# zixunh/vipe

Hardware: AMD Instinct MI355X
Metric: dense-BA+flow update iters/s, 512x384 48-KF graph (higher is better)
Workload: dtype f16 (correlation, GRU; fp32 accumulate) + f32 geometry/BA (fp64 reduced system)

## Files before the change

### include/vipe_amd.h

```cpp
#ifndef VIPE_AMD_H
#define VIPE_AMD_H

#include <stdint.h>

#ifdef __cplusplus
extern "C" {
#endif

#define VIPE_F16 0
#define VIPE_F32 1
#define VIPE_F64 2
#define VIPE_U8 3

#define VIPE_OK 0
#define VIPE_EINVAL (-1)
#define VIPE_ENOSPACE (-2)
#define VIPE_EUNSUPPORTED (-3)

#define VIPE_PYRAMID_REFERENCE 0
#define VIPE_PYRAMID_BLOCKED 1

#define VIPE_CAM_PINHOLE 0
#define VIPE_CAM_MEI 1

// ... 174 lines not shown
int vipe_scatter_mean_rows_f16(const void* d_src, const int64_t* d_ix, void* d_out, int E, int n_out, int64_t inner,
                               void* stream);

int vipe_segment_mean_nhwc_f16(const void* d_src, int src_ctot, int src_coff, const int* d_order, const int* d_rowptr,
                               void* d_out, int n_out, int64_t rows_per_item, int C, void* stream);

int vipe_corr_sampler_forward(const void* d_in1, const void* d_in2, void* d_out, int B, int C, int H, int W, int kH,
                              int kW, int patchH, int patchW, int padH, int padW, int dilH, int dilW,
                              int dil_patchH, int dil_patchW, int dH, int dW, int dtype, void* stream);
int vipe_corr_sampler_backward(const void* d_in1, const void* d_in2, const void* d_grad_out, void* d_grad1,
                               void* d_grad2, int B, int C, int H, int W, int kH, int kW, int patchH, int patchW,
                               int padH, int padW, int dilH, int dilW, int dil_patchH, int dil_patchW, int dH,
                               int dW, int dtype, void* stream);

int vipe_corr_sampler_forward_host(const float* h_in1, const float* h_in2, float* h_out, int B, int C, int H, int W, int kH,
                                   int kW, int patchH, int patchW, int padH, int padW, int dilH, int dilW, int dil_patchH,
                                   int dil_patchW, int dH, int dW);
int vipe_corr_sampler_backward_host(const float* h_in1, const float* h_in2, const float* h_grad_out, float* h_grad1,
                                    float* h_grad2, int B, int C, int H, int W, int kH, int kW, int patchH, int patchW,
                                    int padH, int padW, int dilH, int dilW, int dil_patchH, int dil_patchW, int dH, int dW);

int vipe_nearest_neighbours(const float* d_query, int qdim, const float* d_tree, int tdim, int64_t M, int64_t N, int knn,
                            float* d_dist, int* d_idx, void* stream);

int vipe_ms_deform_attn_forward(const void* d_value, const int64_t* d_spatial_shapes, const int64_t* d_level_start_index,
                                const void* d_sampling_loc, const void* d_attn_weight, void* d_output, int64_t bs,
                                int64_t Lv, int heads, int C, int L, int64_t Lq, int P, int dtype, void* stream);
int vipe_ms_deform_attn_backward(const void* d_value, const int64_t* d_spatial_shapes, const int64_t* d_level_start_index,
                                 const void* d_sampling_loc, const void* d_attn_weight, const void* d_grad_output,
                                 void* d_grad_value, void* d_grad_sampling_loc, void* d_grad_attn_weight, int64_t bs,
                                 int64_t Lv, int heads, int C, int L, int64_t Lq, int P, int dtype, void* stream);

#define VIPE_ACT_NONE 0
#define VIPE_ACT_RELU 1
#define VIPE_ACT_SIGMOID 2
#define VIPE_ACT_TANH 3
int vipe_conv_pack_weights(const void* d_w_oihw, void* d_w_packed, int Cout, int Cin, int KH, int KW, int src_dtype,
                           void* stream);
int vipe_conv2d_nhwc_f16(const void* d_x, const void* d_w_packed, const float* d_bias, const float* d_extra,
                         void* d_y, int B, int H, int W, int Cin, int cin_total, int cin_off, int Cout,
                         int cout_total, int cout_off, int KH, int KW, int act, void* stream);

int vipe_conv_packed_dims(int Cout, int Cin, int KH, int KW, int* cout_pad, int* cin_pad, int* k_pad);

#define VIPE_CONV_PARTIAL 6
#define VIPE_CONV_ACCINIT_F32 0x100
int vipe_conv2d_fused(const void* d_x0, int x0_ctot, int x0_coff, const void* d_x1, int x1_ctot, int x1_coff,
                      int split, const void* d_w_packed, const float* d_bias, const float* d_extra, int extra_stride,
                      int extra_off, void* d_y, int y_ctot, int y_coff, void* d_y2, int y2_ctot, int y2_coff,
                      const void* d_net, int net_ctot, int net_coff, const void* d_z, float* d_fout,
                      const void* d_accinit, int ai_ctot, int ai_coff, int B, int H, int W, int Cin, int Cout, int KH,
                      int KW, int act, int mode, void* stream);

typedef struct {
  const void *corr0_w, *corr2_w, *flow0_w, *flow2_w, *gw_w, *zr_w, *q_w, *zr_s_w, *q_s_w, *heads0_w, *heads2_w, *agg2_w, *eta_w;
  const void *zr_n_w, *zr_x_w;
  const float *corr0_b, *corr2_b, *flow0_b, *flow2_b, *gw_b, *zr_b, *q_b, *heads0_b, *heads2_b, *agg2_b, *eta_b;
  const float* glo_wT;
  const float* glo_b;
} vipe_update_weights;
typedef struct {
  int E, H, W, n_src;
  const void* levels[4];
  const float* coords;
  const int* slots;
  int h2, w2, pyramid_layout;
  const void* corr;
  const void* motn;
  const void* net;
  void* net_out;
  void* xbuf;
  const void* pgate;
  void *c1, *f1, *zb, *rnet;
  void* hbuf;
  float* dw;
  float *glo, *extra;
  const int *order, *rowptr;
  void *agg, *a2;
  float* eta;
  void* side_stream;
  float* pzr;
  int gate_state;
} vipe_update_buffers;
int vipe_update_operator(const vipe_update_weights* weights, const vipe_update_buffers* buffers, void* stream);

int vipe_update_gate_state(const vipe_update_weights* weights, const vipe_update_buffers* buffers, const void* d_net,
                           int parts, void* stream);
typedef struct {
  const vipe_update_weights* weights;
  const vipe_update_buffers* buffers;
  const void* net;
  const int* bounds;
  int n_bounds;
} vipe_gate_state_job;
int vipe_update_gate_state_piece(void* user, int piece, int n_pieces, void* stream);

int vipe_glo_context(const float* d_glo_sum, const float* d_wT, const float* d_bias, float* d_extra, int E, int hw,
                     void* stream);

typedef struct {
  const void* src;
  void* dst;
  const int64_t* idx;
  int64_t src_row_pitch, dst_row_pitch;
  int64_t seg_bytes, seg_pitch;
  int n_seg;
// ... 38 lines not shown
```

### vipe_amd/csrc/conv_mfma.hip

```cpp
#include <stdlib.h>

#include <type_traits>

#include "common.cuh"

namespace {

typedef _Float16 half8 __attribute__((ext_vector_type(8)));
typedef _Float16 half4 __attribute__((ext_vector_type(4)));
typedef float float16v __attribute__((ext_vector_type(16)));
typedef float float4v __attribute__((ext_vector_type(4)));

enum Epi { EPI_PLAIN = 0, EPI_GLO = 1, EPI_ZR = 2, EPI_Q = 3, EPI_HEADS = 4, EPI_ETA = 5, EPI_PARTIAL = 6 };

struct ConvArgs {
  const half_t* x0; int x0_ctot, x0_coff;
  const half_t* x1; int x1_ctot, x1_coff;
  int split;
  const half_t* w;
  const float* bias;
  const float* extra;
  int extra_stride, extra_off;
  half_t* y; int y_ctot, y_coff;
  int B, H, W, Cin, Cin_pad, Cout, Cout_pad, KH, KW, nsteps;
// ... 686 lines not shown
        if (cout0 + tid < a.Cout) atomicAdd(a.fout + (int64_t)e * a.Cout + cout0 + tid, t);
      }
    }
  } else {
    constexpr int PITCH = BMC + 4;
    float* stage = reinterpret_cast<float*>(lds);
#pragma unroll
    for (int i = 0; i < MI; ++i)
#pragma unroll
      for (int j = 0; j < NJ; ++j)
        *reinterpret_cast<float4*>(stage + (wn * 64 + pxh + j * 16 + l16) * PITCH + i * 16 + 4 * lk) =
            make_float4(acc16[i][j][0], acc16[i][j][1], acc16[i][j][2], acc16[i][j][3]);
    __syncthreads();
    float bv[8];
#pragma unroll
    for (int q = 0; q < 8; ++q) {
      bv[q] = a.bias[co + q];
      if (a.extra && co + q < a.Cout) bv[q] += a.extra[(int64_t)e * a.extra_stride + a.extra_off + co + q];
    }
#pragma unroll
    for (int it = 0; it < NIT; ++it) {
      const int pl = pl0 + PSTEP * it;
      const int64_t m = pix_of(pl);
      if (FLAT && m < 0) continue;
      const float4 v0 = *reinterpret_cast<const float4*>(stage + pl * PITCH + ch);
      const float4 v1 = *reinterpret_cast<const float4*>(stage + pl * PITCH + ch + 4);
      const float v[8] = {v0.x + bv[0], v0.y + bv[1], v0.z + bv[2], v0.w + bv[3],
                          v1.x + bv[4], v1.y + bv[5], v1.z + bv[6], v1.w + bv[7]};
      if (a.epi == EPI_HEADS) {
        if (ch == 0)
          *reinterpret_cast<float4*>(a.fout + m * 4) =
              make_float4((float)(half_t)v[0], (float)(half_t)v[1], (float)(half_t)act_apply(v[2], VIPE_ACT_SIGMOID),
                          (float)(half_t)act_apply(v[3], VIPE_ACT_SIGMOID));
      } else if (a.epi == EPI_ETA) {
        if (ch == 0) {
          const float sp = v[0] > 20.0f ? v[0] : log1pf(__expf(v[0]));
          a.fout[m] = 0.01f * (float)(half_t)sp;
        }
      } else {
        half_t* dst = a.y + m * a.y_ctot + a.y_coff + co;
        half8 o;
#pragma unroll
        for (int q = 0; q < 8; ++q) o[q] = (half_t)act_apply(v[q], a.act);
        if (co + 8 <= a.Cout) {
          *reinterpret_cast<half8*>(dst) = o;
        } else {
          for (int q = 0; q < 8 && co + q < a.Cout; ++q) dst[q] = o[q];
        }
      }
    }
  }
}

constexpr int NRW_WBYTES = 9 * 1024;

template <bool FLAT>
__global__ __launch_bounds__(512) __attribute__((amdgpu_waves_per_eu(4, 4))) void conv_halo32_narrow_kernel(ConvArgs a) {
  extern __shared__ __align__(16) unsigned char lds[];
  const int tid = threadIdx.x, lane = tid & 63, wave = __builtin_amdgcn_readfirstlane(tid >> 6);
  const int wn = wave & 3, pxh = (wave >> 2) * 32;
  const int tile = xcd_remap(blockIdx.x, gridDim.x);
  const int xsegs = a.W / HALO_TW, tiles_per_img = FLAT ? a.f_tiles : (a.H / HALO_TH) * xsegs;
  const int e = tile / tiles_per_img, trem = tile % tiles_per_img;
  const int y0 = (trem / xsegs) * HALO_TH, x0 = (trem % xsegs) * HALO_TW;
  const int q0 = trem * (HALO_TH * HALO_TW);
  const int pitch = FLAT ? a.f_wp : HALO_PITCH, xbytes = FLAT ? a.f_xbytes : H32_XBYTES;
  const int npieces = FLAT ? a.f_pieces : H32_PIECES;
  auto pix_of = [&](int pl) -> int64_t {
    if constexpr (FLAT) return flat_pixel(q0 + pl, e, a.H, a.W, a.f_wp, a.f_hwp, a.f_magic);
    else return ((int64_t)(e * a.H + y0 + (pl >> 6))) * a.W + x0 + (pl & 63);
  };
  const int cs32 = a.Cin_pad / H32_BK, cs64 = a.Cin_pad / 64;
  const int r16 = lane >> 2, sl = lane & 3, l16 = lane & 15, lk = lane >> 4;
  const unsigned ldsW_a = lds_address(lds), ldsX_a = ldsW_a + 2 * NRW_WBYTES;
  const unsigned char* ldsW = lds;
  const unsigned char* ldsX = lds + 2 * NRW_WBYTES;
  const half_t* zp = reinterpret_cast<const half_t*>(g_zero_page);

  int xpix[H32_XP];
  const int xk = (sl ^ swzf(r16)) * 8;
#pragma unroll
  for (int i = 0; i < H32_XP; ++i) {
    const int pce = wave + 8 * i;
    const int r = pce * 16 + r16;
    if constexpr (FLAT) {
      xpix[i] = pce < npieces ? flat_pixel(q0 - pitch - 1 + r, e, a.H, a.W, a.f_wp, a.f_hwp, a.f_magic) : -1;
    } else {
      const int hy = r / HALO_PITCH, hx = r % HALO_PITCH;
      const int y = y0 + hy - 1, x = x0 + hx - 1;
      const bool ok = pce < H32_PIECES && r < HALO_ROWS && y >= 0 && y < a.H && x >= 0 && x < a.W;
      xpix[i] = ok ? (e * a.H + y) * a.W + x : -1;
    }
  }
  auto issue = [&](int c, int buf) {
    const int c0 = c * H32_BK;
    const bool s0 = c0 < a.split;
    const int ctot = s0 ? a.x0_ctot : a.x1_ctot;
    const int cb = (s0 ? a.x0_coff : a.x1_coff - a.split) + c0;
#pragma unroll
    for (int i = 0; i < H32_XP; ++i) {
      if (wave + 8 * i < npieces) {
        const bool ok = xpix[i] >= 0 && (c0 + xk < a.Cin);
        const uint64_t off = ((uint64_t)(unsigned)xpix[i] * (unsigned)ctot + (unsigned)(cb + xk)) * 2u;
        const char* src = reinterpret_cast<const char*>(s0 ? a.x0 : a.x1) + off;
        glds16(ok ? (const void*)src : (const void*)zp, ldsX_a + buf * xbytes + (wave + 8 * i) * 1024);
      }
    }
    const unsigned woff = (unsigned)(r16 * 64 + ((sl ^ swzf(r16)) << 3)) * 2u;
    const half_t* wb = a.w + ((int64_t)(wave * cs64 + (c >> 1)) * a.Cout_pad) * BK + (c & 1) * H32_BK;
    glds16_off(wb, woff, ldsW_a + buf * NRW_WBYTES + wave * 1024);
    if (wave == 0) {
      const half_t* w8 = a.w + ((int64_t)(8 * cs64 + (c >> 1)) * a.Cout_pad) * BK + (c & 1) * H32_BK;
      glds16_off(w8, woff, ldsW_a + buf * NRW_WBYTES + 8 * 1024);
    }
  };

  float4v acc[2] = {float4v{0.f, 0.f, 0.f, 0.f}, float4v{0.f, 0.f, 0.f, 0.f}};
  const int wa0 = swz32(l16, lk);
  const int Rl0 = (FLAT ? wn * HALO_TW : wn * HALO_PITCH) + pxh + l16;
  issue(0, 0);
  asm volatile("s_waitcnt vmcnt(0)" ::: "memory");
  __syncthreads();
  for (int c = 0; c < cs32; ++c) {
    if (c + 1 < cs32) issue(c + 1, (c + 1) & 1);
    const unsigned char* bw = ldsW + (c & 1) * NRW_WBYTES;
    const unsigned char* bx = ldsX + (c & 1) * xbytes;
#pragma unroll
    for (int tap = 0; tap < 9; ++tap) {
      const int rb = Rl0 + (tap / 3) * pitch + (tap % 3);
      const int xa0 = swz32(rb, lk);
      const half8 wf = *reinterpret_cast<const half8*>(bw + (wa0 + tap * 1024));
#pragma unroll
      for (int j = 0; j < 2; ++j) {
        const half8 xf = *reinterpret_cast<const half8*>(bx + (xa0 + j * 1024));
        acc[j] = __builtin_amdgcn_mfma_f32_16x16x32_f16(wf, xf, acc[j], 0, 0, 0);
      }
    }
    asm volatile("s_waitcnt vmcnt(0)" ::: "memory");
    __syncthreads();
  }
  constexpr int PITCH = 20;
  float* stage = reinterpret_cast<float*>(lds);
#pragma unroll
  for (int j = 0; j < 2; ++j)
    *reinterpret_cast<float4*>(stage + (wn * 64 + pxh + j * 16 + l16) * PITCH + 4 * lk) =
        make_float4(acc[j][0], acc[j][1], acc[j][2], acc[j][3]);
  __syncthreads();
  const int64_t m = tid < HALO_TH * HALO_TW ? pix_of(tid) : -1;
  if (tid < HALO_TH * HALO_TW && (!FLAT || m >= 0)) {
    float v[16];
#pragma unroll
    for (int q = 0; q < 4; ++q) {
      const float4 t4 = *reinterpret_cast<const float4*>(stage + tid * PITCH + 4 * q);
      v[4 * q] = t4.x; v[4 * q + 1] = t4.y; v[4 * q + 2] = t4.z; v[4 * q + 3] = t4.w;
    }
#pragma unroll
    for (int q = 0; q < 16; ++q) {
      v[q] += a.bias[q];
      if (a.extra && q < a.Cout) v[q] += a.extra[(int64_t)e * a.extra_stride + a.extra_off + q];
    }
    if (a.epi == EPI_HEADS) {
      *reinterpret_cast<float4*>(a.fout + m * 4) =
          make_float4((float)(half_t)v[0], (float)(half_t)v[1], (float)(half_t)act_apply(v[2], VIPE_ACT_SIGMOID),
                      (float)(half_t)act_apply(v[3], VIPE_ACT_SIGMOID));
    } else if (a.epi == EPI_ETA) {
      const float sp = v[0] > 20.0f ? v[0] : log1pf(__expf(v[0]));
      a.fout[m] = 0.01f * (float)(half_t)sp;
    } else {
      half_t* dst = a.y + m * a.y_ctot + a.y_coff;
      for (int q = 0; q < a.Cout; ++q) dst[q] = (half_t)act_apply(v[q], a.act);
    }
  }
}

constexpr int GLO_PITCH = 136;
constexpr size_t GLO_LDS = 256 * GLO_PITCH * 2 + 128 * 4;

__global__ __launch_bounds__(512) __attribute__((amdgpu_waves_per_eu(4, 4))) void conv1x1_glo_kernel(ConvArgs a) {
  extern __shared__ __align__(16) unsigned char lds[];
  half_t* xt = reinterpret_cast<half_t*>(lds);
  float* gacc = reinterpret_cast<float*>(lds + 256 * GLO_PITCH * 2);
  const int tid = threadIdx.x, lane = tid & 63, wave = tid >> 6;
  const int l16 = lane & 15, kg = lane >> 4;
  const int wq = wave & 3, wp = wave >> 2;
  const int HW = a.H * a.W;
  const int tpi = (HW + 255) / 256;
  const int e = blockIdx.x / tpi, p0 = (blockIdx.x % tpi) * 256;
  const int64_t pix0 = (int64_t)e * HW + p0;
  if (tid < 128) gacc[tid] = 0.0f;
#pragma unroll
  for (int it = 0; it < 8; ++it) {
    const int i = tid + 512 * it, px = i >> 4, ck = i & 15;
    half8 v = {0, 0, 0, 0, 0, 0, 0, 0};
// ... 206 lines not shown
  if (vipe_conv_packed_dims(Cout, Cin, KH, KW, &cp, &cinp, &kp) != VIPE_OK) return VIPE_EINVAL;
  VIPE_CHECK_ARG(Cin == 4 || Cin % 8 == 0);
  const int64_t total = (int64_t)kp * cp;
  pack_weights_kernel<<<(int)std::min<int64_t>((total + 255) / 256, 4096), 256, 0, as_stream(stream)>>>(
      d_w_oihw, (half_t*)d_w_packed, Cout, Cin, KH, KW, cp, cinp, kp, src_dtype == VIPE_F32, Cin == 4);
  return vipe_launch_status();
}

}

namespace {

template <typename K>
void allow_lds(K kernel, std::atomic<uint64_t>& seen, size_t bytes) {
  vipe_once_per_device(seen, [&] { (void)hipFuncSetAttribute((const void*)kernel, hipFuncAttributeMaxDynamicSharedMemorySize, (int)bytes); });
}
constexpr size_t MAX_LDS = 160 * 1024;

bool flat_geometry(ConvArgs& a, int pad) {
  a.f_wp = a.W + pad;
  a.f_hwp = a.H * a.f_wp;
  a.f_tiles = (a.f_hwp + 255) / 256;
  a.f_magic = (unsigned)(((1ull << 32) + (unsigned)a.f_wp - 1) / (unsigned)a.f_wp);
  const int rows = 256 + 2 * a.f_wp + 2;
  a.f_pieces = (rows + 15) / 16;
  a.f_xbytes = a.f_pieces * 1024;
  a.f_p1lo = (a.f_wp + 1) / 16;
  a.f_p1hi = (a.f_wp + 256) / 16;
  return a.f_wp >= 2 && a.f_pieces <= 8 * H32_XP && a.f_hwp < (1 << 23);
}

inline bool needs_tile_kernel(const ConvArgs& a) { return a.accinit || a.epi == EPI_PARTIAL || a.ai_f32; }

template <int BMC, int KS, int VAR, bool FLAT>
int launch_halo32(const ConvArgs& a, int tiles, int gy, size_t lds, hipStream_t s) {
  static std::atomic<uint64_t> seen{0};
  allow_lds(conv_halo32_kernel<BMC, KS, true, VAR, FLAT>, seen, FLAT ? MAX_LDS : lds);
  conv_halo32_kernel<BMC, KS, true, VAR, FLAT><<<dim3(tiles * gy), 512, lds, s>>>(a, gy);
  return vipe_launch_status();
}

template <bool FLAT>
int launch_halo_family(ConvArgs& a, int cp, int64_t M, hipStream_t s) {
  const bool split_ok = a.split >= a.Cin || a.split % H32_BK == 0;
  const int tiles = FLAT ? a.B * a.f_tiles : (int)(M / (HALO_TH * HALO_TW));
  const size_t xb = FLAT ? (size_t)a.f_xbytes : (size_t)H32_XBYTES;
  if (needs_tile_kernel(a)) {
    const bool ok = cp >= 64 && split_ok && !(a.KH == 3 && a.Cout <= 16) && !(a.epi == EPI_PARTIAL && a.Cout % 4 != 0) &&
                    !(a.ai_f32 && !a.accinit);
    if (!ok) return VIPE_EUNSUPPORTED;
  }
  if (a.KH == 3 && a.Cout <= 16 && cp == 32 && split_ok && (a.epi == EPI_HEADS || a.epi == EPI_ETA || a.epi == EPI_PLAIN)) {
    static std::atomic<uint64_t> seen{0};
    const size_t lds = 2 * NRW_WBYTES + 2 * xb + 1024;
    allow_lds(conv_halo32_narrow_kernel<FLAT>, seen, FLAT ? MAX_LDS : lds);
    conv_halo32_narrow_kernel<FLAT><<<dim3(tiles), 512, lds, s>>>(a);
    return vipe_launch_status();
  }
  if (!split_ok) return VIPE_EUNSUPPORTED;
  const int bmc = cp >= 128 ? 128 : cp;
  const int gy = cp >= 128 ? cp / 128 : 1;
  size_t lds = 3 * (size_t)bmc * 64 + 2 * xb + 1024;
  const size_t stage = bmc >= 64 ? (size_t)256 * (bmc + 8) * 2 : (size_t)256 * 36 * 4;
  if (lds < stage) lds = stage;
  if (a.ai_f32 || a.epi == EPI_PARTIAL) {
    if (!(a.KH == 3 && bmc == 128 && !(a.ai_f32 && a.epi == EPI_PARTIAL))) return VIPE_EUNSUPPORTED;
    return a.ai_f32 ? launch_halo32<128, 3, 1, FLAT>(a, tiles, gy, lds, s) : launch_halo32<128, 3, 2, FLAT>(a, tiles, gy, lds, s);
  }
  if (a.KH == 3) {
    if (bmc == 128) return launch_halo32<128, 3, 0, FLAT>(a, tiles, gy, lds, s);
    if (bmc == 64) return launch_halo32<64, 3, 0, FLAT>(a, tiles, 1, lds, s);
    return launch_halo32<32, 3, 0, FLAT>(a, tiles, 1, lds, s);
  }
  if (bmc == 128) return launch_halo32<128, 1, 0, FLAT>(a, tiles, gy, lds, s);
  if (bmc == 64) return launch_halo32<64, 1, 0, FLAT>(a, tiles, 1, lds, s);
  return launch_halo32<32, 1, 0, FLAT>(a, tiles, 1, lds, s);
}

int launch_conv(ConvArgs& a, hipStream_t s) {
  int cp, cinp, kp;
  if (vipe_conv_packed_dims(a.Cout, a.Cin, a.KH, a.KW, &cp, &cinp, &kp) != VIPE_OK) return VIPE_EINVAL;
  a.Cout_pad = cp;
  a.Cin_pad = cinp;
  a.nsteps = kp / 64;
  const int64_t M = (int64_t)a.B * a.H * a.W;
  if (M == 0) return VIPE_OK;
  const bool small = a.Cin == 4;
  const int gx = (int)((M + BNP - 1) / BNP);
  const bool sq13 = !small && a.KH == a.KW && (a.KH == 1 || a.KH == 3);
  const bool off32 = (int64_t)a.B * a.H * a.W < (1ll << 31);
  const bool aligned = a.W % HALO_TW == 0 && a.H % HALO_TH == 0;
  const bool halo = sq13 && aligned && off32;
  const bool flat = sq13 && !aligned && off32 && flat_geometry(a, a.KH == 3 ? 1 : 0);
  if (needs_tile_kernel(a) && !halo && !flat) return VIPE_EUNSUPPORTED;
  if (a.epi == EPI_GLO && a.KH == 1 && a.KW == 1 && a.Cin == 128 && a.Cout == 128 && cp == 128 && a.split >= a.Cin &&
      a.x0_ctot % 8 == 0 && a.x0_coff % 8 == 0 && a.net == a.x0 && a.net_ctot == a.x0_ctot && a.net_coff == a.x0_coff &&
      a.extra == nullptr) {
    static std::atomic<uint64_t> seen{0};
    allow_lds(conv1x1_glo_kernel, seen, GLO_LDS);
    conv1x1_glo_kernel<<<dim3((unsigned)(a.B * ((a.H * a.W + 255) / 256))), 512, GLO_LDS, s>>>(a);
    return vipe_launch_status();
  }
  if (halo) {
    const int rc = launch_halo_family<false>(a, cp, M, s);
    if (rc != VIPE_EUNSUPPORTED || needs_tile_kernel(a)) return rc;
  } else if (flat) {
    const int rc = launch_halo_family<true>(a, cp, M, s);
    if (rc != VIPE_EUNSUPPORTED || needs_tile_kernel(a)) return rc;
  }
  if (small && a.KH == 7 && a.KW == 7 && cp % 128 == 0 && kp == 256 && a.epi == EPI_PLAIN && a.extra == nullptr &&
      (int64_t)a.B * a.H * a.W < (1ll << 31)) {
    const int gy = cp / 128;
    if (aligned) {
      static std::atomic<uint64_t> seen{0};
      allow_lds(conv7x7_c4_kernel<false>, seen, C7_LDS);
      conv7x7_c4_kernel<false><<<dim3((int)(M / (HALO_TH * HALO_TW)) * gy), 512, C7_LDS, s>>>(a, gy);
      return vipe_launch_status();
    }
    flat_geometry(a, 3);
    const size_t need = C7_WBYTES + (size_t)(256 + 6 * a.f_wp + 6) * 8;
    if (need <= MAX_LDS && a.f_hwp < (1 << 23) && a.f_wp >= 2) {
      static std::atomic<uint64_t> seen{0};
      allow_lds(conv7x7_c4_kernel<true>, seen, MAX_LDS);
      const size_t lds = need > (size_t)(256 * 136 * 2) ? need : (size_t)(256 * 136 * 2);
      conv7x7_c4_kernel<true><<<dim3(a.B * a.f_tiles * gy), 512, lds, s>>>(a, gy);
      return vipe_launch_status();
    }
  }
  const bool glds = !small && a.KH * a.KW <= 32;
  static std::atomic<uint64_t> s1{0}, s2{0}, s3{0};
  allow_lds(conv_mfma_kernel<128, 2, 2, false>, s1, 65536);
  allow_lds(conv_mfma_kernel<128, 2, 2, true>, s2, 65536);
  allow_lds(conv_mfma_glds_kernel<128, 2, 2>, s3, 65536);
  if (cp >= 128) {
    const size_t lds = 2 * (128 + BNP) * 128;
// ... 30 lines not shown
  VIPE_CHECK_ARG(Cin == 4 || (cin_total % 8 == 0 && cin_off % 8 == 0));
  VIPE_CHECK_ARG(act >= 0 && act <= 3);
  ConvArgs a = {};
  a.x0 = (const half_t*)d_x; a.x0_ctot = cin_total; a.x0_coff = cin_off;
  a.x1 = a.x0; a.x1_ctot = cin_total; a.x1_coff = cin_off; a.split = Cin;
  a.w = (const half_t*)d_w_packed; a.bias = d_bias; a.extra = d_extra; a.extra_stride = Cout; a.extra_off = 0;
  a.y = (half_t*)d_y; a.y_ctot = cout_total; a.y_coff = cout_off;
  a.B = B; a.H = H; a.W = W; a.Cin = Cin; a.Cout = Cout; a.KH = KH; a.KW = KW;
  a.act = act; a.epi = EPI_PLAIN;
  return launch_conv(a, as_stream(stream));
}

VIPE_EXPORT int vipe_conv2d_fused(const void* d_x0, int x0_ctot, int x0_coff, const void* d_x1, int x1_ctot,
                                  int x1_coff, int split, const void* d_w_packed, const float* d_bias,
                                  const float* d_extra, int extra_stride, int extra_off, void* d_y, int y_ctot,
                                  int y_coff, void* d_y2, int y2_ctot, int y2_coff, const void* d_net, int net_ctot,
                                  int net_coff, const void* d_z, float* d_fout, const void* d_accinit, int ai_ctot,
                                  int ai_coff, int B, int H, int W, int Cin, int Cout, int KH, int KW, int act, int mode,
                                  void* stream) {
  VIPE_CHECK_ARG(d_x0 && d_w_packed && d_bias);
  VIPE_CHECK_ARG(!d_accinit || (ai_ctot % 4 == 0 && ai_coff % 4 == 0 && ai_coff + Cout <= ai_ctot));
  VIPE_CHECK_ARG(B >= 0 && H > 0 && W > 0 && Cin > 0 && Cout > 0 && (KH & 1) && (KW & 1));
  if (Cin == 4) {
    VIPE_CHECK_ARG(split >= Cin && x0_ctot % 4 == 0 && x0_coff % 4 == 0);
  } else {
    VIPE_CHECK_ARG(Cin % 8 == 0 && x0_ctot % 8 == 0 && x0_coff % 8 == 0);
    VIPE_CHECK_ARG(split >= Cin || (split % 64 == 0 && d_x1 && x1_ctot % 8 == 0 && x1_coff % 8 == 0));
  }
  const int ai_f32 = (mode & VIPE_CONV_ACCINIT_F32) != 0;
  mode &= ~VIPE_CONV_ACCINIT_F32;
  VIPE_CHECK_ARG(mode >= EPI_PLAIN && mode <= EPI_PARTIAL);
  if (mode == EPI_PARTIAL) VIPE_CHECK_ARG(d_fout && y_ctot % 4 == 0 && y_coff % 4 == 0 && y_coff + Cout <= y_ctot && !d_extra);
  if (mode == EPI_PLAIN) VIPE_CHECK_ARG(d_y && y_ctot % 4 == 0 && y_coff % 4 == 0);
  if (mode == EPI_GLO) VIPE_CHECK_ARG(d_net && d_fout);
  if (mode == EPI_ZR) VIPE_CHECK_ARG(d_y && d_y2 && d_net && Cout == 256);
  if (mode == EPI_Q) VIPE_CHECK_ARG(d_y && d_net && d_z && Cout == 128);
  if (mode == EPI_HEADS) VIPE_CHECK_ARG(d_fout && Cout == 4);
  if (mode == EPI_ETA) VIPE_CHECK_ARG(d_fout && Cout == 1);
  ConvArgs a = {};
  a.x0 = (const half_t*)d_x0; a.x0_ctot = x0_ctot; a.x0_coff = x0_coff;
  a.x1 = (const half_t*)(d_x1 ? d_x1 : d_x0); a.x1_ctot = d_x1 ? x1_ctot : x0_ctot; a.x1_coff = d_x1 ? x1_coff : x0_coff;
  a.split = split > Cin ? Cin : split;
  a.w = (const half_t*)d_w_packed; a.bias = d_bias; a.extra = d_extra; a.extra_stride = extra_stride; a.extra_off = extra_off;
  a.y = (half_t*)d_y; a.y_ctot = y_ctot; a.y_coff = y_coff;
  a.y2 = (half_t*)d_y2; a.y2_ctot = y2_ctot; a.y2_coff = y2_coff;
  a.net = (const half_t*)d_net; a.net_ctot = net_ctot; a.net_coff = net_coff;
  a.zbuf = (const half_t*)d_z; a.fout = d_fout;
  a.accinit = (const half_t*)d_accinit; a.ai_ctot = ai_ctot; a.ai_coff = ai_coff; a.ai_f32 = ai_f32;
  a.B = B; a.H = H; a.W = W; a.Cin = Cin; a.Cout = Cout; a.KH = KH; a.KW = KW;
  a.act = act; a.epi = mode;
  return launch_conv(a, as_stream(stream));
}

}
```

### vipe_amd/csrc/update_op.hip

```cpp
#include "common.cuh"

namespace {

__global__ __launch_bounds__(384) void glo_gemm_kernel(const float* __restrict__ glo, const float* __restrict__ wT ,
                                                       const float* __restrict__ b, float* __restrict__ extra, float inv_hw) {
  __shared__ float g[128];
  const int e = blockIdx.x, t = threadIdx.x;
  if (t < 128) g[t] = glo[(int64_t)e * 128 + t] * inv_hw;
  __syncthreads();
  float acc = b[t];
#pragma unroll 8
  for (int k = 0; k < 128; ++k) acc = __builtin_fmaf(g[k], wT[k * 384 + t], acc);
  extra[(int64_t)e * 384 + t] = acc;
}

__global__ __launch_bounds__(256) void update_finish_kernel(const float* __restrict__ coords1, const float* __restrict__ dw,
                                                            const unsigned char* __restrict__ mask, float* __restrict__ target,
                                                            float* __restrict__ weight, const float* __restrict__ eta,
                                                            const int64_t* __restrict__ du, float* __restrict__ damping,
                                                            int64_t n_px, int64_t n_eta, int P) {
  const int64_t i = (int64_t)blockIdx.x * 256 + threadIdx.x;
  if (i < n_px) {
    const float2 c = reinterpret_cast<const float2*>(coords1)[i];
    const float4 d = reinterpret_cast<const float4*>(dw)[i];
    const bool m = mask && mask[i];
    reinterpret_cast<float2*>(target)[i] = make_float2(c.x + d.x, c.y + d.y);
    reinterpret_cast<float2*>(weight)[i] = m ? make_float2(0.f, 0.f) : make_float2(d.z, d.w);
  }
  if (i < n_eta) damping[du[i / P] * P + i % P] = eta[i];
}

}

namespace {
hipEvent_t* operator_events() {
  static thread_local hipEvent_t ev[64][4] = {};
  int d = 0;
  (void)hipGetDevice(&d);
  hipEvent_t* e = ev[d & 63];
  for (int i = 0; i < 4; ++i)
    if (!e[i] && hipEventCreateWithFlags(&e[i], hipEventDisableTiming) != hipSuccess) return nullptr;
  return e;
}
}

extern "C" {

VIPE_EXPORT int vipe_update_operator(const vipe_update_weights* wt, const vipe_update_buffers* b, void* stream) {
  VIPE_CHECK_ARG(wt && b && b->E >= 0 && b->H > 0 && b->W > 0);
  if (b->E == 0) return VIPE_OK;
  const int E = b->E, H = b->H, W = b->W;
  hipStream_t s = as_stream(stream);
  int rc;
#define RUN(call)              \
  do {                         \
    rc = (call);               \
    if (rc != VIPE_OK) return rc; \
  } while (0)
  hipStream_t s2 = (hipStream_t)b->side_stream;
  hipEvent_t* ev = s2 ? operator_events() : nullptr;
  if (s2 && !ev) return VIPE_EINVAL;
  void* const stream2 = s2 ? b->side_stream : stream;
#define FORK(i)                                                                                              \
  do {                                                                                                       \
    if (s2 && (hipEventRecord(ev[i], s) != hipSuccess || hipStreamWaitEvent(s2, ev[i], 0) != hipSuccess)) return VIPE_EINVAL; \
  } while (0)
#define JOIN(i)                                                                                              \
  do {                                                                                                       \
    if (s2 && (hipEventRecord(ev[i], s2) != hipSuccess || hipStreamWaitEvent(s, ev[i], 0) != hipSuccess)) return VIPE_EINVAL; \
  } while (0)
  FORK(0);
  if (b->levels[0]) {
    RUN(vipe_corr_lookup_conv1x1(b->levels, b->coords, wt->corr0_w, wt->corr0_b, b->c1, 128, 0, E, H, W, b->h2, b->w2, 128,
                                 VIPE_ACT_RELU, b->slots, b->pyramid_layout, stream));
  } else {
    VIPE_CHECK_ARG(b->corr);
    RUN(vipe_conv2d_fused(b->corr, 200, 0, nullptr, 0, 0, 200, wt->corr0_w, wt->corr0_b, nullptr, 0, 0, b->c1, 128, 0, nullptr,
                          0, 0, nullptr, 0, 0, nullptr, nullptr, nullptr, 0, 0, E, H, W, 200, 128, 1, 1, VIPE_ACT_RELU, 0, stream));
  }
  RUN(vipe_conv2d_fused(b->c1, 128, 0, nullptr, 0, 0, 128, wt->corr2_w, wt->corr2_b, nullptr, 0, 0, b->xbuf, 320, 128, nullptr,
                        0, 0, nullptr, 0, 0, nullptr, nullptr, nullptr, 0, 0, E, H, W, 128, 128, 3, 3, VIPE_ACT_RELU, 0, stream));
  RUN(vipe_conv2d_fused(b->motn, 4, 0, nullptr, 0, 0, 4, wt->flow0_w, wt->flow0_b, nullptr, 0, 0, b->f1, 128, 0, nullptr, 0, 0,
                        nullptr, 0, 0, nullptr, nullptr, nullptr, 0, 0, E, H, W, 4, 128, 7, 7, VIPE_ACT_RELU, 0, stream2));
  RUN(vipe_conv2d_fused(b->f1, 128, 0, nullptr, 0, 0, 128, wt->flow2_w, wt->flow2_b, nullptr, 0, 0, b->xbuf, 320, 256, nullptr,
                        0, 0, nullptr, 0, 0, nullptr, nullptr, nullptr, 0, 0, E, H, W, 128, 64, 3, 3, VIPE_ACT_RELU, 0, stream2));
  JOIN(1);
  const int Es = b->gate_state;
  const bool staged = Es != 0;
  if (staged) VIPE_CHECK_ARG(Es > 0 && Es <= E && b->pgate && b->pzr && wt->zr_x_w);
  if (!staged) {
    if (hipMemsetAsync(b->glo, 0, sizeof(float) * 128 * (size_t)E, s) != hipSuccess) return VIPE_EINVAL;
    RUN(vipe_conv2d_fused(b->net, 128, 0, nullptr, 0, 0, 128, wt->gw_w, wt->gw_b, nullptr, 0, 0, nullptr, 0, 0, nullptr, 0, 0,
                          b->net, 128, 0, nullptr, b->glo, nullptr, 0, 0, E, H, W, 128, 128, 1, 1, VIPE_ACT_NONE, 1, stream));
    glo_gemm_kernel<<<E, 384, 0, s>>>(b->glo, wt->glo_wT, wt->glo_b, b->extra, 1.0f / (float)(H * W));
  }
  if (staged) {
    RUN(vipe_conv2d_fused(b->xbuf, 320, 128, nullptr, 0, 0, 192, wt->zr_x_w, wt->zr_b, b->extra, 384, 0, b->zb, 128, 0, b->rnet,
                          128, 0, b->net, 128, 0, nullptr, nullptr, b->pzr, 256, 0, Es, H, W, 192, 256, 3, 3, VIPE_ACT_NONE,
                          2 | VIPE_CONV_ACCINIT_F32, stream));
    if (Es < E) {
      const int64_t px = (int64_t)Es * H * W;
      auto h16 = [&](const void* p, int c) { return (const void*)((const char*)p + px * c * 2); };
      RUN(vipe_conv2d_fused(h16(b->net, 128), 128, 0, h16(b->xbuf, 320), 320, 128, 128, wt->zr_s_w, wt->zr_b,
                            b->extra + (int64_t)Es * 384, 384, 0, (void*)h16(b->zb, 128), 128, 0, (void*)h16(b->rnet, 128), 128, 0,
                            h16(b->net, 128), 128, 0, nullptr, nullptr, h16(b->pgate, 384), 384, 0, E - Es, H, W, 320, 256, 3, 3,
                            VIPE_ACT_NONE, 2, stream));
    }
    RUN(vipe_conv2d_fused(b->rnet, 128, 0, b->xbuf, 320, 128, 128, wt->q_s_w, wt->q_b, b->extra, 384, 256, b->net_out, 128, 0,
                          nullptr, 0, 0, b->net, 128, 0, b->zb, nullptr, b->pgate, 384, 256, E, H, W, 320, 128, 3, 3,
                          VIPE_ACT_NONE, 3, stream));
  } else if (b->pgate) {
    RUN(vipe_conv2d_fused(b->net, 128, 0, b->xbuf, 320, 128, 128, wt->zr_s_w, wt->zr_b, b->extra, 384, 0, b->zb, 128, 0, b->rnet,
                          128, 0, b->net, 128, 0, nullptr, nullptr, b->pgate, 384, 0, E, H, W, 320, 256, 3, 3, VIPE_ACT_NONE, 2,
                          stream));
    RUN(vipe_conv2d_fused(b->rnet, 128, 0, b->xbuf, 320, 128, 128, wt->q_s_w, wt->q_b, b->extra, 384, 256, b->net_out, 128, 0,
                          nullptr, 0, 0, b->net, 128, 0, b->zb, nullptr, b->pgate, 384, 256, E, H, W, 320, 128, 3, 3,
                          VIPE_ACT_NONE, 3, stream));
  } else {
    RUN(vipe_conv2d_fused(b->net, 128, 0, b->xbuf, 320, 0, 128, wt->zr_w, wt->zr_b, b->extra, 384, 0, b->zb, 128, 0, b->rnet, 128,
                          0, b->net, 128, 0, nullptr, nullptr, nullptr, 0, 0, E, H, W, 448, 256, 3, 3, VIPE_ACT_NONE, 2, stream));
    RUN(vipe_conv2d_fused(b->rnet, 128, 0, b->xbuf, 320, 0, 128, wt->q_w, wt->q_b, b->extra, 384, 256, b->net_out, 128, 0, nullptr,
                          0, 0, b->net, 128, 0, b->zb, nullptr, nullptr, 0, 0, E, H, W, 448, 128, 3, 3, VIPE_ACT_NONE, 3, stream));
  }
  RUN(vipe_conv2d_fused(b->net_out, 128, 0, nullptr, 0, 0, 128, wt->heads0_w, wt->heads0_b, nullptr, 0, 0, b->hbuf, 384, 0,
                        nullptr, 0, 0, nullptr, 0, 0, nullptr, nullptr, nullptr, 0, 0, E, H, W, 128, 384, 3, 3, VIPE_ACT_RELU, 0,
                        stream));
  const bool two_tails = s2 && b->n_src > 0;
  if (two_tails) FORK(2);
  RUN(vipe_conv2d_fused(b->hbuf, 384, 0, nullptr, 0, 0, 256, wt->heads2_w, wt->heads2_b, nullptr, 0, 0, nullptr, 0, 0, nullptr, 0,
                        0, nullptr, 0, 0, nullptr, b->dw, nullptr, 0, 0, E, H, W, 256, 4, 3, 3, VIPE_ACT_NONE, 4,
                        two_tails ? stream2 : stream));
  if (b->n_src > 0) {
    VIPE_CHECK_ARG(b->order && b->rowptr && b->agg && b->a2 && b->eta);
    RUN(vipe_segment_mean_nhwc_f16(b->hbuf, 384, 256, b->order, b->rowptr, b->agg, b->n_src, (int64_t)H * W, 128, stream));
    RUN(vipe_conv2d_fused(b->agg, 128, 0, nullptr, 0, 0, 128, wt->agg2_w, wt->agg2_b, nullptr, 0, 0, b->a2, 128, 0, nullptr, 0, 0,
                          nullptr, 0, 0, nullptr, nullptr, nullptr, 0, 0, b->n_src, H, W, 128, 128, 3, 3, VIPE_ACT_RELU, 0,
                          stream));
    RUN(vipe_conv2d_fused(b->a2, 128, 0, nullptr, 0, 0, 128, wt->eta_w, wt->eta_b, nullptr, 0, 0, nullptr, 0, 0, nullptr, 0, 0,
                          nullptr, 0, 0, nullptr, b->eta, nullptr, 0, 0, b->n_src, H, W, 128, 1, 3, 3, VIPE_ACT_NONE, 5, stream));
  }
  if (two_tails) JOIN(3);
#undef FORK
#undef JOIN
#undef RUN
  return vipe_launch_status();
}

VIPE_EXPORT int vipe_update_gate_state(const vipe_update_weights* wt, const vipe_update_buffers* b, const void* d_net,
                                       int parts, void* stream) {
  VIPE_CHECK_ARG(wt && b && b->E >= 0 && b->H > 0 && b->W > 0 && parts >= 1 && parts <= 3);
  if (b->E == 0) return VIPE_OK;
  VIPE_CHECK_ARG(d_net && (!(parts & 1) || (b->glo && b->extra)) && (!(parts & 2) || (b->pgate && b->pzr && wt->zr_n_w)));
  const int E = b->E, H = b->H, W = b->W;
  hipStream_t s = as_stream(stream);
  int rc;
  if (parts & 1) {
    if (hipMemsetAsync(b->glo, 0, sizeof(float) * 128 * (size_t)E, s) != hipSuccess) return VIPE_EINVAL;
    rc = vipe_conv2d_fused(d_net, 128, 0, nullptr, 0, 0, 128, wt->gw_w, wt->gw_b, nullptr, 0, 0, nullptr, 0, 0, nullptr, 0, 0,
                           d_net, 128, 0, nullptr, b->glo, nullptr, 0, 0, E, H, W, 128, 128, 1, 1, VIPE_ACT_NONE, 1, stream);
    if (rc != VIPE_OK) return rc;
    glo_gemm_kernel<<<E, 384, 0, s>>>(b->glo, wt->glo_wT, wt->glo_b, b->extra, 1.0f / (float)(H * W));
  }
  if (parts & 2) {
    rc = vipe_conv2d_fused(d_net, 128, 0, nullptr, 0, 0, 128, wt->zr_n_w, wt->zr_b, nullptr, 0, 0, nullptr, 256, 0, nullptr, 0,
                           0, nullptr, 0, 0, nullptr, b->pzr, b->pgate, 384, 0, E, H, W, 128, 256, 3, 3, VIPE_ACT_NONE,
                           VIPE_CONV_PARTIAL, stream);
    if (rc != VIPE_OK) return rc;
  }
  return vipe_launch_status();
}

VIPE_EXPORT int vipe_update_gate_state_piece(void* user, int piece, int n_pieces, void* stream) {
  const vipe_gate_state_job* j = (const vipe_gate_state_job*)user;
  VIPE_CHECK_ARG(j && j->weights && j->buffers && j->net && n_pieces > 0 && piece >= 0 && piece < n_pieces);
  const vipe_update_buffers* b = j->buffers;
  VIPE_CHECK_ARG(b->E >= 0 && b->H > 0 && b->W > 0 && b->pgate && b->pzr);
  int64_t e0 = (int64_t)b->E * piece / n_pieces, e1 = (int64_t)b->E * (piece + 1) / n_pieces;
  if (j->bounds && j->n_bounds == n_pieces + 1) {
    e0 = j->bounds[piece];
    e1 = j->bounds[piece + 1];
    VIPE_CHECK_ARG(j->bounds[0] == 0 && j->bounds[n_pieces] == b->E && e0 >= 0 && e0 <= e1 && e1 <= b->E);
  }
  if (e1 <= e0) return VIPE_OK;
  const int64_t px = (int64_t)b->H * b->W;
  vipe_update_buffers sub = *b;
  sub.E = (int)(e1 - e0);
  sub.pgate = (const char*)b->pgate + e0 * px * 384 * 2;
  sub.pzr = b->pzr + e0 * px * 256;
  return vipe_update_gate_state(j->weights, &sub, (const char*)j->net + e0 * px * 128 * 2, 2, stream);
}

VIPE_EXPORT int vipe_glo_context(const float* d_glo_sum, const float* d_wT, const float* d_bias, float* d_extra, int E, int hw,
// ... 24 lines not shown
```

Before: 250.6.

## Split heads0 conv by output channels to overlap aggregation tail; register-resident narrow weights

The heads0 conv is split into two output-channel blocks through a new cout_block entry point. The aggregation chain (segment mean, agg2, eta), which only reads channels 256-383, can then fork onto the second stream right after that block, while channels 0-255 and heads2 run on the main stream. Separately, the narrow-Cout halo conv now loads its weights straight into registers with scalar-based global loads instead of staging them in LDS. It also uses a three-slot LDS ring for the input halo with partial vmcnt waits, so prefetch runs further ahead. This trades more register pressure, an extra launch and hand-written waitcnt immediates for better overlap.

```diff
diff --git a/include/vipe_amd.h b/include/vipe_amd.h
--- a/include/vipe_amd.h
+++ b/include/vipe_amd.h
@@ -250,6 +250,10 @@
                       const void* d_accinit, int ai_ctot, int ai_coff, int B, int H, int W, int Cin, int Cout, int KH,
                       int KW, int act, int mode, void* stream);
 
+int vipe_conv2d_cout_block(const void* d_x, int x_ctot, int x_coff, const void* d_w_packed, const float* d_bias, void* d_y,
+                           int y_ctot, int y_coff, int B, int H, int W, int Cin, int cout_full, int cout_lo, int cout_n,
+                           int KH, int KW, int act, void* stream);
+
 typedef struct {
   const void *corr0_w, *corr2_w, *flow0_w, *flow2_w, *gw_w, *zr_w, *q_w, *zr_s_w, *q_s_w, *heads0_w, *heads2_w, *agg2_w, *eta_w;
   const void *zr_n_w, *zr_x_w;
diff --git a/vipe_amd/csrc/conv_mfma.hip b/vipe_amd/csrc/conv_mfma.hip
--- a/vipe_amd/csrc/conv_mfma.hip
+++ b/vipe_amd/csrc/conv_mfma.hip
@@ -762,7 +762,25 @@
   }
 }
 
-constexpr int NRW_WBYTES = 9 * 1024;
+constexpr int NRW_RING = 3;
+constexpr int NRW_XQ = H32_XP;
+static_assert(NRW_XQ == 4, "conv_halo32_narrow_kernel's s_waitcnt immediates are written for 4 halo DMAs per wave and chunk");
+
+__device__ __forceinline__ half8 gload16s(uint64_t sbase, unsigned voff_bytes) {
+  half8 v = {0, 0, 0, 0, 0, 0, 0, 0};
+#if defined(__HIP_DEVICE_COMPILE__)
+  asm volatile("global_load_dwordx4 %0, %1, %2" : "=v"(v) : "v"(voff_bytes), "s"(sbase) : "memory");
+#endif
+  return v;
+}
+__device__ __forceinline__ void nrw_wait(half8 (&w)[9]) {
+#if defined(__HIP_DEVICE_COMPILE__)
+  asm volatile("s_waitcnt vmcnt(4)"
+               : "+v"(w[0]), "+v"(w[1]), "+v"(w[2]), "+v"(w[3]), "+v"(w[4]), "+v"(w[5]), "+v"(w[6]), "+v"(w[7]), "+v"(w[8])
+               :
+               : "memory");
+#endif
+}
 
 template <bool FLAT>
 __global__ __launch_bounds__(512) __attribute__((amdgpu_waves_per_eu(4, 4))) void conv_halo32_narrow_kernel(ConvArgs a) {
@@ -782,10 +800,11 @@
   };
   const int cs32 = a.Cin_pad / H32_BK, cs64 = a.Cin_pad / 64;
   const int r16 = lane >> 2, sl = lane & 3, l16 = lane & 15, lk = lane >> 4;
-  const unsigned ldsW_a = lds_address(lds), ldsX_a = ldsW_a + 2 * NRW_WBYTES;
-  const unsigned char* ldsW = lds;
-  const unsigned char* ldsX = lds + 2 * NRW_WBYTES;
-  const half_t* zp = reinterpret_cast<const half_t*>(g_zero_page);
+  const unsigned ldsX_a = lds_address(lds);
+  const unsigned ldsX_u = __builtin_amdgcn_readfirstlane(ldsX_a + wave * 1024);
+  const unsigned sink_u = __builtin_amdgcn_readfirstlane(ldsX_a + NRW_RING * xbytes);
+  const unsigned char* ldsX = lds;
+  const uint64_t zp64 = uniform64((uint64_t)g_zero_page);
 
   int xpix[H32_XP];
   const int xk = (sl ^ swzf(r16)) * 8;
@@ -802,53 +821,64 @@
       xpix[i] = ok ? (e * a.H + y) * a.W + x : -1;
     }
   }
-  auto issue = [&](int c, int buf) {
+  const uint64_t xbase0 = uniform64((uint64_t)a.x0), xbase1 = uniform64((uint64_t)a.x1);
+  auto issueX = [&](int c, int slot, bool on) {
     const int c0 = c * H32_BK;
     const bool s0 = c0 < a.split;
     const int ctot = s0 ? a.x0_ctot : a.x1_ctot;
     const int cb = (s0 ? a.x0_coff : a.x1_coff - a.split) + c0;
+    const uint64_t base = s0 ? xbase0 : xbase1;
 #pragma unroll
     for (int i = 0; i < H32_XP; ++i) {
-      if (wave + 8 * i < npieces) {
-        const bool ok = xpix[i] >= 0 && (c0 + xk < a.Cin);
-        const uint64_t off = ((uint64_t)(unsigned)xpix[i] * (unsigned)ctot + (unsigned)(cb + xk)) * 2u;
-        const char* src = reinterpret_cast<const char*>(s0 ? a.x0 : a.x1) + off;
-        glds16(ok ? (const void*)src : (const void*)zp, ldsX_a + buf * xbytes + (wave + 8 * i) * 1024);
-      }
-    }
-    const unsigned woff = (unsigned)(r16 * 64 + ((sl ^ swzf(r16)) << 3)) * 2u;
-    const half_t* wb = a.w + ((int64_t)(wave * cs64 + (c >> 1)) * a.Cout_pad) * BK + (c & 1) * H32_BK;
-    glds16_off(wb, woff, ldsW_a + buf * NRW_WBYTES + wave * 1024);
-    if (wave == 0) {
-      const half_t* w8 = a.w + ((int64_t)(8 * cs64 + (c >> 1)) * a.Cout_pad) * BK + (c & 1) * H32_BK;
-      glds16_off(w8, woff, ldsW_a + buf * NRW_WBYTES + 8 * 1024);
-    }
+      const bool real = on && (wave + 8 * i < npieces);
+      const bool ok = real && xpix[i] >= 0 && (c0 + xk < a.Cin);
+      const uint64_t off = ((uint64_t)(unsigned)xpix[i] * (unsigned)ctot + (unsigned)(cb + xk)) * 2u;
+      const unsigned dst = real ? ldsX_u + (unsigned)(slot * xbytes + i * 8192) : sink_u;
+      dma16v(ok ? base + off : zp64, __builtin_amdgcn_readfirstlane(dst));
+    }
+  };
+  const uint64_t wbase = uniform64((uint64_t)a.w);
+  const int wrows = a.Cout <= 1 ? 1 : a.Cout <= 2 ? 2 : a.Cout <= 4 ? 4 : a.Cout <= 8 ? 8 : 16;
+  const unsigned wvoff = (unsigned)((l16 & (wrows - 1)) * BK + lk * 8) * 2u;
+  const unsigned tstride = (unsigned)cs64 * (unsigned)a.Cout_pad * BK * 2u;
+  auto loadW = [&](int c, half8 (&w)[9]) {
+    const uint64_t b = wbase + (uint64_t)(((unsigned)(c >> 1) * (unsigned)a.Cout_pad * BK + (unsigned)(c & 1) * H32_BK) * 2u);
+#pragma unroll
+    for (int tap = 0; tap < 9; ++tap) w[tap] = gload16s(b + (uint64_t)((unsigned)tap * tstride), wvoff);
   };
 
   float4v acc[2] = {float4v{0.f, 0.f, 0.f, 0.f}, float4v{0.f, 0.f, 0.f, 0.f}};
-  const int wa0 = swz32(l16, lk);
   const int Rl0 = (FLAT ? wn * HALO_TW : wn * HALO_PITCH) + pxh + l16;
-  issue(0, 0);
-  asm volatile("s_waitcnt vmcnt(0)" ::: "memory");
+  half8 wc[9], wnx[9];
+  issueX(0, 0, true);
+  loadW(0, wc);
+  issueX(1, 1, cs32 > 1);
+  nrw_wait(wc);
   __syncthreads();
+  int slot = 0;
   for (int c = 0; c < cs32; ++c) {
-    if (c + 1 < cs32) issue(c + 1, (c + 1) & 1);
-    const unsigned char* bw = ldsW + (c & 1) * NRW_WBYTES;
-    const unsigned char* bx = ldsX + (c & 1) * xbytes;
+    loadW(c + 1 < cs32 ? c + 1 : c, wnx);
+    const int slot2 = slot == 0 ? 2 : slot - 1;
+    issueX(c + 2, slot2, c + 2 < cs32);
+    const unsigned char* bx = ldsX + slot * xbytes;
 #pragma unroll
     for (int tap = 0; tap < 9; ++tap) {
       const int rb = Rl0 + (tap / 3) * pitch + (tap % 3);
       const int xa0 = swz32(rb, lk);
-      const half8 wf = *reinterpret_cast<const half8*>(bw + (wa0 + tap * 1024));
 #pragma unroll
       for (int j = 0; j < 2; ++j) {
         const half8 xf = *reinterpret_cast<const half8*>(bx + (xa0 + j * 1024));
-        acc[j] = __builtin_amdgcn_mfma_f32_16x16x32_f16(wf, xf, acc[j], 0, 0, 0);
+        acc[j] = __builtin_amdgcn_mfma_f32_16x16x32_f16(wc[tap], xf, acc[j], 0, 0, 0);
       }
     }
-    asm volatile("s_waitcnt vmcnt(0)" ::: "memory");
+    nrw_wait(wnx);
     __syncthreads();
-  }
+#pragma unroll
+    for (int tap = 0; tap < 9; ++tap) wc[tap] = wnx[tap];
+    slot = slot == 2 ? 0 : slot + 1;
+  }
+  asm volatile("s_waitcnt vmcnt(0)" ::: "memory");
+  __syncthreads();
   constexpr int PITCH = 20;
   float* stage = reinterpret_cast<float*>(lds);
 #pragma unroll
@@ -1161,7 +1191,7 @@
   }
   if (a.KH == 3 && a.Cout <= 16 && cp == 32 && split_ok && (a.epi == EPI_HEADS || a.epi == EPI_ETA || a.epi == EPI_PLAIN)) {
     static std::atomic<uint64_t> seen{0};
-    const size_t lds = 2 * NRW_WBYTES + 2 * xb + 1024;
+    const size_t lds = NRW_RING * xb + 1024;
     allow_lds(conv_halo32_narrow_kernel<FLAT>, seen, FLAT ? MAX_LDS : lds);
     conv_halo32_narrow_kernel<FLAT><<<dim3(tiles), 512, lds, s>>>(a);
     return vipe_launch_status();
@@ -1186,10 +1216,10 @@
   return launch_halo32<32, 1, 0, FLAT>(a, tiles, 1, lds, s);
 }
 
-int launch_conv(ConvArgs& a, hipStream_t s) {
+int launch_conv(ConvArgs& a, hipStream_t s, int w_rows = 0) {
   int cp, cinp, kp;
   if (vipe_conv_packed_dims(a.Cout, a.Cin, a.KH, a.KW, &cp, &cinp, &kp) != VIPE_OK) return VIPE_EINVAL;
-  a.Cout_pad = cp;
+  a.Cout_pad = w_rows ? w_rows : cp;
   a.Cin_pad = cinp;
   a.nsteps = kp / 64;
   const int64_t M = (int64_t)a.B * a.H * a.W;
@@ -1326,4 +1356,23 @@
   return launch_conv(a, as_stream(stream));
 }
 
-}
+VIPE_EXPORT int vipe_conv2d_cout_block(const void* d_x, int x_ctot, int x_coff, const void* d_w_packed, const float* d_bias,
+                                       void* d_y, int y_ctot, int y_coff, int B, int H, int W, int Cin, int cout_full,
+                                       int cout_lo, int cout_n, int KH, int KW, int act, void* stream) {
+  VIPE_CHECK_ARG(d_x && d_w_packed && d_bias && d_y);
+  VIPE_CHECK_ARG(B >= 0 && H > 0 && W > 0 && Cin > 0 && Cin % 8 == 0 && (KH & 1) && (KW & 1));
+  VIPE_CHECK_ARG(x_ctot % 8 == 0 && x_coff % 8 == 0 && y_ctot % 4 == 0 && y_coff % 4 == 0 && act >= 0 && act <= 3);
+  VIPE_CHECK_ARG(cout_lo >= 0 && cout_n > 0 && cout_lo % 128 == 0 && cout_n % 128 == 0 && cout_lo + cout_n <= cout_full);
+  int cp_full;
+  if (vipe_conv_packed_dims(cout_full, Cin, KH, KW, &cp_full, nullptr, nullptr) != VIPE_OK) return VIPE_EINVAL;
+  ConvArgs a = {};
+  a.x0 = (const half_t*)d_x; a.x0_ctot = x_ctot; a.x0_coff = x_coff;
+  a.x1 = a.x0; a.x1_ctot = x_ctot; a.x1_coff = x_coff; a.split = Cin;
+  a.w = (const half_t*)d_w_packed + (int64_t)cout_lo * BK; a.bias = d_bias + cout_lo;
+  a.y = (half_t*)d_y; a.y_ctot = y_ctot; a.y_coff = y_coff + cout_lo;
+  a.B = B; a.H = H; a.W = W; a.Cin = Cin; a.Cout = cout_n; a.KH = KH; a.KW = KW;
+  a.act = act; a.epi = EPI_PLAIN;
+  return launch_conv(a, as_stream(stream), cp_full);
+}
+
+}
diff --git a/vipe_amd/csrc/update_op.hip b/vipe_amd/csrc/update_op.hip
--- a/vipe_amd/csrc/update_op.hip
+++ b/vipe_amd/csrc/update_op.hip
@@ -1,3 +1,6 @@
+#include <stdlib.h>
+#include <string.h>
+
 #include "common.cuh"
 
 namespace {
@@ -41,6 +44,16 @@
   for (int i = 0; i < 4; ++i)
     if (!e[i] && hipEventCreateWithFlags(&e[i], hipEventDisableTiming) != hipSuccess) return nullptr;
   return e;
+}
+}
+
+namespace {
+bool tail_agg_first() {
+  static const bool v = [] {
+    const char* e = getenv("VIPE_AMD_OP_TAIL_ORDER");
+    return !(e && strcmp(e, "heads") == 0);
+  }();
+  return v;
 }
 }
 
@@ -122,22 +135,37 @@
     RUN(vipe_conv2d_fused(b->rnet, 128, 0, b->xbuf, 320, 0, 128, wt->q_w, wt->q_b, b->extra, 384, 256, b->net_out, 128, 0, nullptr,
                           0, 0, b->net, 128, 0, b->zb, nullptr, nullptr, 0, 0, E, H, W, 448, 128, 3, 3, VIPE_ACT_NONE, 3, stream));
   }
-  RUN(vipe_conv2d_fused(b->net_out, 128, 0, nullptr, 0, 0, 128, wt->heads0_w, wt->heads0_b, nullptr, 0, 0, b->hbuf, 384, 0,
-                        nullptr, 0, 0, nullptr, 0, 0, nullptr, nullptr, nullptr, 0, 0, E, H, W, 128, 384, 3, 3, VIPE_ACT_RELU, 0,
-                        stream));
+  auto heads0_block = [&](int lo, int n) {
+    return vipe_conv2d_cout_block(b->net_out, 128, 0, wt->heads0_w, wt->heads0_b, b->hbuf, 384, 0, E, H, W, 128, 384, lo, n, 3, 3,
+                                  VIPE_ACT_RELU, stream);
+  };
+  auto heads2 = [&](void* st) {
+    return vipe_conv2d_fused(b->hbuf, 384, 0, nullptr, 0, 0, 256, wt->heads2_w, wt->heads2_b, nullptr, 0, 0, nullptr, 0, 0, nullptr,
+                             0, 0, nullptr, 0, 0, nullptr, b->dw, nullptr, 0, 0, E, H, W, 256, 4, 3, 3, VIPE_ACT_NONE, 4, st);
+  };
+  auto agg_chain = [&](void* st) {
+    int r = vipe_segment_mean_nhwc_f16(b->hbuf, 384, 256, b->order, b->rowptr, b->agg, b->n_src, (int64_t)H * W, 128, st);
+    if (r != VIPE_OK) return r;
+    r = vipe_conv2d_fused(b->agg, 128, 0, nullptr, 0, 0, 128, wt->agg2_w, wt->agg2_b, nullptr, 0, 0, b->a2, 128, 0, nullptr, 0, 0,
+                          nullptr, 0, 0, nullptr, nullptr, nullptr, 0, 0, b->n_src, H, W, 128, 128, 3, 3, VIPE_ACT_RELU, 0, st);
+    if (r != VIPE_OK) return r;
+    return vipe_conv2d_fused(b->a2, 128, 0, nullptr, 0, 0, 128, wt->eta_w, wt->eta_b, nullptr, 0, 0, nullptr, 0, 0, nullptr, 0, 0,
+                             nullptr, 0, 0, nullptr, b->eta, nullptr, 0, 0, b->n_src, H, W, 128, 1, 3, 3, VIPE_ACT_NONE, 5, st);
+  };
+  if (b->n_src > 0) VIPE_CHECK_ARG(b->order && b->rowptr && b->agg && b->a2 && b->eta);
   const bool two_tails = s2 && b->n_src > 0;
-  if (two_tails) FORK(2);
-  RUN(vipe_conv2d_fused(b->hbuf, 384, 0, nullptr, 0, 0, 256, wt->heads2_w, wt->heads2_b, nullptr, 0, 0, nullptr, 0, 0, nullptr, 0,
-                        0, nullptr, 0, 0, nullptr, b->dw, nullptr, 0, 0, E, H, W, 256, 4, 3, 3, VIPE_ACT_NONE, 4,
-                        two_tails ? stream2 : stream));
-  if (b->n_src > 0) {
-    VIPE_CHECK_ARG(b->order && b->rowptr && b->agg && b->a2 && b->eta);
-    RUN(vipe_segment_mean_nhwc_f16(b->hbuf, 384, 256, b->order, b->rowptr, b->agg, b->n_src, (int64_t)H * W, 128, stream));
-    RUN(vipe_conv2d_fused(b->agg, 128, 0, nullptr, 0, 0, 128, wt->agg2_w, wt->agg2_b, nullptr, 0, 0, b->a2, 128, 0, nullptr, 0, 0,
-                          nullptr, 0, 0, nullptr, nullptr, nullptr, 0, 0, b->n_src, H, W, 128, 128, 3, 3, VIPE_ACT_RELU, 0,
-                          stream));
-    RUN(vipe_conv2d_fused(b->a2, 128, 0, nullptr, 0, 0, 128, wt->eta_w, wt->eta_b, nullptr, 0, 0, nullptr, 0, 0, nullptr, 0, 0,
-                          nullptr, 0, 0, nullptr, b->eta, nullptr, 0, 0, b->n_src, H, W, 128, 1, 3, 3, VIPE_ACT_NONE, 5, stream));
+  if (tail_agg_first()) {
+    RUN(heads0_block(256, 128));
+    if (two_tails) FORK(2);
+    RUN(heads0_block(0, 256));
+    RUN(heads2(stream));
+    if (b->n_src > 0) RUN(agg_chain(two_tails ? stream2 : stream));
+  } else {
+    RUN(heads0_block(0, 256));
+    if (two_tails) FORK(2);
+    RUN(heads2(two_tails ? stream2 : stream));
+    RUN(heads0_block(256, 128));
+    if (b->n_src > 0) RUN(agg_chain(stream));
   }
   if (two_tails) JOIN(3);
 #undef FORK
```

Result: slower. 241.4 (-3.7%).
